# xiaosu-zhu/McQuic

Measured on AMD Instinct MI355X. Metric: images/sec encode+decode, 768x512 Kodak-shape batch, qp=2, higher is better.
Workload: dtype f32; 1 GPU; qp=2 reference model Compressor(128, 2, [8192, 2048, 512]), batch=32 768x512 random images per GPU, encode+decode tensor path (BASELINE configs[1]); images_per_gpu=32, parallelism=dp1 (independent image shards, no data-path collective)

## Files before the change

mcquic_amd/csrc/conv_launch.hip:

```cpp
#include <mutex>
#include <unordered_map>

#include "conv_instances.h"
#include "conv_sizes.h"
#include "conv_wino16.h"
#include "conv_head16.h"
#include "conv_t16.h"

namespace {

std::mutex g_sec_mu;
bool g_sec_trace = false;
std::unordered_map<const float*, unsigned> g_sec_used;
inline void sec_note(const mcq_conv_desc* descs, int nprob, unsigned bit) {
    if (!g_sec_trace) return;
    std::lock_guard<std::mutex> lock(g_sec_mu);
    for (int c = 0; c < nprob; ++c) g_sec_used[descs[c].w_packed] |= bit;
}

bool wino_shape(int Cout, int ksize, int stride, unsigned fl) {
    return ksize == 3 && stride == 1 && Cout % 64 == 0 && !(fl & (MCQ_CONV_SILU_IN | MCQ_CONV_SQUARE_IN));
}

inline bool post_fills_chip(long long tb, int row_tiles) { return tb * row_tiles >= 2048; }

int block_width_log2(int rows, int cols, int min_lg) {
    int best_log2 = 5; double best_util = -1.0;
    for (int lg = 5; lg >= min_lg; --lg) {
        const int bw = 1 << lg, bh = 32 >> lg;
        const double cover = (double)((rows + bh - 1) / bh * bh) * (double)((cols + bw - 1) / bw * bw);
        const double util = (double)rows * cols / cover;
        if (util > best_util + 1e-9) { best_util = util; best_log2 = lg; }
    }
    return best_log2;
}

template <class P> void conv_ptrs(P& a, const mcq_conv_desc* e, size_t sec4, size_t sec2) {
    a.x = e->x; a.wp = e->w_packed; a.wp64 = a.wp + sec4; a.wp32 = a.wp64 + sec2;
    a.bias = e->bias; a.y = e->y; a.y2 = e->y_silu; a.res = e->res; a.mul = e->mul; a.gid = e->gate_id;
}
template <class P> void w16_ptrs(P& a, const mcq_conv_desc* e) {
    a.x = e->x; a.wp = e->w_packed; a.bias = e->bias; a.y = e->y; a.y2 = e->y_silu; a.res = e->res;
}
void t16_ptrs(T16Ptrs& a, const mcq_conv_desc* e, size_t sec) {
    a.x = e->x; a.wp = e->w_packed + sec; a.bias = e->bias; a.y = e->y; a.y2 = e->y_silu; a.res = e->res; a.mul = e->mul;
}

int conv_validate(const mcq_conv_desc* d) {
    if (!d || !d->x || !d->w_packed || !d->y) return MCQ_EINVAL;
    if (d->N <= 0 || d->Cin <= 0 || d->H <= 0 || d->W <= 0 || d->Cout <= 0) return MCQ_EINVAL;
    if ((d->ksize != 1 && d->ksize != 3) || (d->stride != 1 && d->stride != 2)) return MCQ_EINVAL;
    if ((d->flags & MCQ_CONV_TAPS_LR) && (d->ksize != 3 || d->stride != 1 || (d->flags & (MCQ_CONV_WINOGRAD | MCQ_CONV_WINOGRAD2D | MCQ_CONV_WINOGRAD2D16 |
                                                                                    MCQ_CONV_SILU_IN | MCQ_CONV_SQUARE_IN)))) return MCQ_EINVAL;
    const unsigned fl = d->flags & ~(unsigned)MCQ_CONV_TAPS_LR;
    if (fl & MCQ_CONV_POST_MASK) {
        const unsigned post = fl & MCQ_CONV_POST_MASK;
        if ((post & (post - 1)) || !d->post_w || d->ksize != 3 || (d->flags & MCQ_CONV_TAPS_LR)) return MCQ_EINVAL;
        unsigned allowed = MCQ_CONV_POST_MASK | MCQ_CONV_SILU_IN;
        if (post == MCQ_CONV_POST_IGDN) allowed |= MCQ_CONV_SHUFFLE2;
        if (post == MCQ_CONV_POST_GATE) allowed |= MCQ_CONV_RESIDUAL | MCQ_CONV_DUAL_SILU;
        if (fl & ~allowed) return MCQ_EINVAL;
        if (d->Cout != ((fl & MCQ_CONV_SHUFFLE2) ? 512 : 128)) return MCQ_EINVAL;
        if (post == MCQ_CONV_POST_GATE && (!d->mul || !d->gate_id || d->stride != 1)) return MCQ_EINVAL;
    }
    if ((fl & MCQ_CONV_RESIDUAL) && !d->res) return MCQ_EINVAL;
    if ((fl & (MCQ_CONV_GDN | MCQ_CONV_IGDN | MCQ_CONV_GATE | MCQ_CONV_MUL | MCQ_CONV_DSILU_MUL)) && !d->mul) return MCQ_EINVAL;
    if ((fl & MCQ_CONV_GATE) && !d->gate_id) return MCQ_EINVAL;
    if ((fl & MCQ_CONV_DUAL_SILU) && (!d->y_silu || (fl & MCQ_CONV_SILU_OUT))) return MCQ_EINVAL;
    if (fl & (MCQ_CONV_GDN_BWD | MCQ_CONV_IGDN_BWD)) {
        if (!d->res || !d->mul || !d->y_silu || (fl & ~(unsigned)(MCQ_CONV_SQUARE_IN | MCQ_CONV_GDN_BWD | MCQ_CONV_IGDN_BWD)) ||
            (fl & MCQ_CONV_GDN_BWD && fl & MCQ_CONV_IGDN_BWD) || d->ksize != 1) return MCQ_EINVAL;
    }
    if (fl & MCQ_CONV_GATE_BWD) {
        if (!d->res || !d->mul || !d->y_silu || (fl & ~(unsigned)MCQ_CONV_GATE_BWD) || d->ksize != 1 || d->stride != 1) return MCQ_EINVAL;
    }
    if ((fl & MCQ_CONV_SILU_IN) && (fl & MCQ_CONV_SQUARE_IN)) return MCQ_EINVAL;
    if (fl & MCQ_CONV_SHUFFLE2) {
        if ((d->Cout & 3) || (fl & ~(unsigned)(MCQ_CONV_SHUFFLE2 | MCQ_CONV_SILU_IN | MCQ_CONV_SQUARE_IN | MCQ_CONV_WINOGRAD | MCQ_CONV_WINOGRAD2D | MCQ_CONV_WINOGRAD2D16 |
                                               MCQ_CONV_DSILU_MUL | MCQ_CONV_RESIDUAL | MCQ_CONV_POST_IGDN))) return MCQ_EINVAL;
        if ((fl & (MCQ_CONV_DSILU_MUL | MCQ_CONV_RESIDUAL)) && (fl & (MCQ_CONV_WINOGRAD | MCQ_CONV_WINOGRAD2D | MCQ_CONV_WINOGRAD2D16)))
            return MCQ_EINVAL;
    }
    if ((uint64_t)(d->Cin + 8) * d->H * d->W * 4ull >= 0x80000000ull) return MCQ_ETOOLARGE;
    return MCQ_OK;
}

bool t16_takes(int N, int Cin, int H, int W, int Cout, int ksize, int stride, unsigned fl, int nprob) {
    return N > 0 && H > 0 && W > 0 && nprob >= 1 && t16_shape(Cout, Cin, ksize) && stride == 1 && (fl & ~T16_FLAGS) == 0 &&
           t16_tiles((long long)N * H * W, Cout, nprob) <= T16_MAX_TILES &&
// ... 20 lines not shown
    for (int c = 1; c < MCQ_CONV_MAX_MULTI; ++c) conv_ptrs(k.alt[c - 1], descs + (c < nprob ? c : 0), sec4, sec2);

    if (fl & MCQ_CONV_WINOGRAD2D16) {
        if ((fl & (MCQ_CONV_WINOGRAD | MCQ_CONV_WINOGRAD2D)) || !wino_shape(d->Cout, d->ksize, d->stride, fl)) return MCQ_EINVAL;
        W16K w;
        w16_ptrs(w, d);
        for (int c = 1; c < W16_MAX_MULTI; ++c) w16_ptrs(w.alt[c - 1], descs + (c < nprob ? c : 0));
        w.nprob = nprob; w.N = d->N; w.Cin = d->Cin; w.H = d->H; w.W = d->W; w.Cout = d->Cout; w.Ho = k.Ho; w.Wo = k.Wo;
        w.flags = fl & ~(unsigned)MCQ_CONV_WINOGRAD2D16; w.res_scale = d->res_scale;
        return mcq_wino16_launch(w, stream);
    }
    if (fl & MCQ_CONV_WINOGRAD2D) {
        if ((fl & MCQ_CONV_WINOGRAD) || !wino_shape(d->Cout, d->ksize, d->stride, fl) || d->Cout % 128 != 0 || d->Cin % 8 != 0) return MCQ_EINVAL;
        if ((uint64_t)(d->Cin + 16) * d->H * d->W * 4ull >= 0x80000000ull) return MCQ_ETOOLARGE;
        k.TP = k.S * 16;
        k.wp32 = k.wp; k.wp64 = k.wp;
        for (int c = 1; c < MCQ_CONV_MAX_MULTI; ++c) { k.alt[c - 1].wp32 = k.alt[c - 1].wp; k.alt[c - 1].wp64 = k.alt[c - 1].wp; }
        const int Wt = (k.Wo + 1) / 2, Ht = (k.Ho + 1) / 2;
        const int best_log2 = block_width_log2(Ht, Wt, 0);
        k.bw_log2 = best_log2;
        k.nbx = (Wt + (1 << best_log2) - 1) >> best_log2;
        k.nby = (Ht + (32 >> best_log2) - 1) / (32 >> best_log2);
        const long long tbw = (long long)k.N * k.nbx * k.nby;
        if (tbw > 0x7fffffffLL) return MCQ_ETOOLARGE;
        k.total_blocks = (int)tbw;
        if ((uint64_t)d->Cout * (uint64_t)k.Ho * k.Wo * 4ull >= 0x80000000ull) return MCQ_ETOOLARGE;
        k.flags = fl & ~(unsigned)MCQ_CONV_WINOGRAD2D;
        return launch_wino2d(k, tbw, d->Cout / 128, (hipStream_t)stream);
    }
    if (fl & MCQ_CONV_WINOGRAD) {
        if (!wino_shape(d->Cout, d->ksize, d->stride, fl)) return MCQ_EINVAL;
        if ((uint64_t)(d->Cin + 16) * d->H * d->W * 4ull >= 0x80000000ull) return MCQ_ETOOLARGE;
        const int forced_mb = (d->tile & 0xff) >> 4;
        const int MBw = forced_mb == 2 || d->Cout % 128 != 0 ? 2 : 4;
        k.TP = k.S * 12;
        k.wp64 = k.wp + wino_section_floats(d->Cout, d->Cin, 4);
        k.wp32 = k.wp64;
        for (int c = 1; c < MCQ_CONV_MAX_MULTI; ++c) {
            k.alt[c - 1].wp64 = k.alt[c - 1].wp + wino_section_floats(d->Cout, d->Cin, 4);
            k.alt[c - 1].wp32 = k.alt[c - 1].wp64;
        }
        const int Wp = (k.Wo + 1) / 2;
        const int best_log2 = block_width_log2(k.Ho, Wp, 2);
        k.bw_log2 = best_log2;
        k.nbx = (Wp + (1 << best_log2) - 1) >> best_log2;
        k.nby = (k.Ho + (32 >> best_log2) - 1) / (32 >> best_log2);
        const long long tbw = (long long)k.N * k.nbx * k.nby;
        if (tbw > 0x7fffffffLL) return MCQ_ETOOLARGE;
        k.total_blocks = (int)tbw;
        const int co_tiles = (d->Cout + 32 * MBw - 1) / (32 * MBw);
        if ((uint64_t)co_tiles * 32u * (unsigned)MBw * (uint64_t)k.Ho * k.Wo * 4ull >= 0x80000000ull) return MCQ_ETOOLARGE;
        k.flags = fl & ~(unsigned)MCQ_CONV_WINOGRAD;
        return MBw == 4 ? launch_wino<4>(k, tbw, co_tiles, (hipStream_t)stream) : launch_wino<2>(k, tbw, co_tiles, (hipStream_t)stream);
    }

    if (d->tile == 0 && t16_takes(d->N, d->Cin, d->H, d->W, d->Cout, d->ksize, d->stride, fl, nprob)) {
        sec_note(descs, nprob, 8u);
        T16K t;
        const size_t sec = section_floats(d->Cout, d->Cin, 3, 4) + section_floats(d->Cout, d->Cin, 3, 2) + section_floats(d->Cout, d->Cin, 3, 1);
        for (int c = 0; c < MCQ_CONV_MAX_MULTI; ++c) t16_ptrs(t.p[c], descs + (c < nprob ? c : 0), sec);
        t.N = d->N; t.Cin = d->Cin; t.H = d->H; t.W = d->W; t.Cout = d->Cout; t.flags = fl; t.res_scale = d->res_scale;
        const dim3 grid((unsigned)(((long long)d->N * d->H * d->W + 15) / 16), (unsigned)(d->Cout / 16), (unsigned)nprob);
        if (d->Cin == 128) hipLaunchKernelGGL(conv_t16_kernel<8>, grid, dim3(256), 0, (hipStream_t)stream, t);
        else hipLaunchKernelGGL(conv_t16_kernel<4>, grid, dim3(256), 0, (hipStream_t)stream, t);
        return mcq_check_launch();
    }

    if (nprob == 1 && head16_shape(d->Cout, d->ksize) && d->stride == 1 && (d->tile & 0xff) == 0 &&
        (fl & ~(unsigned)(MCQ_CONV_SHUFFLE2 | MCQ_CONV_SILU_IN)) == 0) {
        if ((uint64_t)d->Cout * d->H * d->W * 4ull >= 0x80000000ull) return MCQ_ETOOLARGE;
        Head16K h;
        h.x = d->x; h.wp16 = d->w_packed + general_floats(d->Cout, d->Cin, d->ksize); h.bias = d->bias; h.y = d->y;
        h.N = d->N; h.Cin = d->Cin; h.H = d->H; h.W = d->W; h.Cout = d->Cout;
        h.S4 = (d->Cin + 3) / 4;
        h.gpr = (d->W + 15) / 16;
        h.total_groups = (long long)d->N * d->H * h.gpr;
        h.flags = fl;
        const long long waves = (h.total_groups + H16_NB - 1) / H16_NB;
        if ((waves + 3) / 4 > 0x7fffffffLL) return MCQ_ETOOLARGE;
        const dim3 grid((unsigned)((waves + 3) / 4));
        if (fl & MCQ_CONV_SILU_IN) hipLaunchKernelGGL(conv_head16_kernel<PRO_SILU>, grid, dim3(256), 0, (hipStream_t)stream, h);
        else hipLaunchKernelGGL(conv_head16_kernel<PRO_NONE>, grid, dim3(256), 0, (hipStream_t)stream, h);
        return mcq_check_launch();
    }

    const int best_log2 = block_width_log2(k.Ho, k.Wo, 2);
    k.bw_log2 = best_log2;
    const int bw = 1 << best_log2, bh = 32 >> best_log2;
    k.nbx = (k.Wo + bw - 1) / bw;
    k.nby = (k.Ho + bh - 1) / bh;
    const long long tb = (long long)k.N * k.nbx * k.nby;
    if (tb > 0x7fffffffLL) return MCQ_ETOOLARGE;
    k.total_blocks = (int)tb;

    const int co32 = (d->Cout + 31) / 32;
    int MB, NB, ksl = 0;
    bool dsilu41 = false;
    const int forced = d->tile & 0xff;
    if (forced) {
        MB = forced >> 4; NB = forced & 15; ksl = (d->tile >> 8) & 3;
        if ((MB != 1 && MB != 2 && MB != 4) || (NB != 1 && NB != 2 && NB != 4)) return MCQ_EINVAL;
    }
    else if (co32 == 1) {
        MB = 1; NB = (tb * nprob >= 4 * 2048) ? 4 : 2;
        if (d->Cin <= 64) {
            NB = (tb * nprob >= 16384) ? 2 : 1;
            while (ksl < 3 && (((tb + NB - 1) / NB * nprob) << ksl) < 1024) ++ksl;
        }
    }
    else if (co32 == 2 && ((tb + 1) / 2) * nprob < 2048 && d->ksize == 3) {
        MB = 1; NB = 1;
        while (ksl < 3 && ((tb * co32 * nprob) << ksl) < 1024) ++ksl;
    }
    else {
        static const int cand[3][2] = {{4, 2}, {2, 2}, {1, 1}};
        MB = 1; NB = 1;
        const bool rows64 = ((co32 + 3) / 4) * 4 > ((co32 + 1) / 2) * 2;
        for (int c = 0; c < 3; ++c) {
            const int mb = cand[c][0], nb = cand[c][1];
            if (mb > co32 || (mb == 4 && rows64)) continue;
            const long long tiles = ((tb + nb - 1) / nb) * ((co32 + mb - 1) / mb);
            MB = mb; NB = nb;
            if (tiles * 8 >= 1024) break;
        }
        const long long tiles1 = ((tb + NB - 1) / NB) * ((co32 + MB - 1) / MB);
        const long long tiles = tiles1 * nprob;
        while (ksl < 3 && (tiles << ksl) < 2048) ++ksl;
        int ksl1 = 0;
        while (ksl1 < 3 && (tiles1 << ksl1) < 2048) ++ksl1;
        if (MB == 4 && NB == 2 && ksl1 == 2 && tiles1 * 4 > 2048 && tiles1 * 4 <= 3072 && d->ksize == 3 &&
            k.S % 2 == 0 && (k.S >> 1) >= 8) { MB = 2; NB = 2; ksl = nprob >= 2 ? 0 : 1; }
        if (MB == 4 && NB == 2 && ksl == 3 && d->ksize == 3 && k.S % 4 == 0 && (k.S >> 2) >= 8) { NB = 1; ksl = 2; }
        else if (MB == 4 && NB == 2 && ksl == 1 && d->ksize == 3) { NB = 1; ksl = 0; }
        else if (MB == 4 && NB == 2 && ksl == 2 && nprob >= 2 && d->ksize == 3 && k.S % 2 == 0 && (k.S >> 1) >= 8) { MB = 2; ksl = 1; }
        else if (MB == 4 && NB == 2 && ksl == 0 && (fl & MCQ_CONV_DSILU_MUL) && d->ksize == 3) { NB = 1; dsilu41 = true; }
        if (d->ksize == 1 && d->stride == 1 && co32 >= 4) {
            const long long t41 = tb * ((co32 + 3) / 4) * nprob, t21 = tb * ((co32 + 1) / 2) * nprob;
            if (t41 >= 2048 && !rows64) { MB = 4; NB = 1; ksl = 0; }
            else if (t21 >= 2048) { MB = 2; NB = 1; ksl = 0; }
        }
    }
    if (fl & (MCQ_CONV_GDN_BWD | MCQ_CONV_IGDN_BWD)) {
        if (!(fl & MCQ_CONV_SQUARE_IN)) return MCQ_EINVAL;
        NB = 1; ksl = 0;
    }
    if (fl & MCQ_CONV_GATE_BWD) { NB = 1; ksl = 0; }
    int post = 0;
    if (fl & MCQ_CONV_POST_MASK) {
        if (nprob != 1 || lr4) return MCQ_EINVAL;
        if (!post_fills_chip(tb, (fl & MCQ_CONV_SHUFFLE2) ? 4 : 1) && forced != 0x41) return MCQ_EINVAL;
        MB = 4; NB = 1; ksl = 0; dsilu41 = false;
        post = (fl & MCQ_CONV_POST_GATE) ? 2 : 1;
        k.post_sub = (fl & MCQ_CONV_SHUFFLE2) ? 1 : 0;
    }
    const int pro = (fl & MCQ_CONV_SILU_IN) ? PRO_SILU : (fl & MCQ_CONV_SQUARE_IN) ? PRO_SQUARE : PRO_NONE;
    long long ptiles = (tb + NB - 1) / NB;
    const bool pair_ok = !post && !lr4 && MB == 4 && (NB == 2 || dsilu41) && ksl == 0 && d->ksize == 3 && d->stride == 1 && pro == PRO_NONE && (k.Wo & 1) == 0 &&
                         !(fl & ~(unsigned)(MCQ_CONV_SILU_OUT | MCQ_CONV_RESIDUAL | MCQ_CONV_DUAL_SILU | MCQ_CONV_DSILU_MUL | MCQ_CONV_SHUFFLE2));
    const bool pair = pair_ok && (d->tile & 0x400);
    if (pair) {
        const int Wp = k.Wo / 2;
        const int bl = block_width_log2(k.Ho, Wp, 2);
        const int pnbx = (Wp + (1 << bl) - 1) >> bl, pnby = (k.Ho + (32 >> bl) - 1) / (32 >> bl);
        const long long pt = (long long)k.N * pnbx * pnby;
        NB = 2; k.bw_log2 = bl; k.nbx = pnbx; k.nby = pnby; ptiles = pt; k.total_blocks = (int)pt;
    }
// ... 71 lines not shown
```

mcquic_amd/modules/compressor.py:

```python
from __future__ import annotations

import operator
from typing import List, Tuple

import torch
import torch.nn.functional as F
from torch import nn

from ..nn import AttentionBlock, ResidualBlock, ResidualBlockShuffle, ResidualBlockWithStride, conv3x3, pixelShuffle3x3
from ..utils.specification import FileHeader, ImageSize
from .quantizer import BaseQuantizer, ResidualBackwardQuantizer, UMGMQuantizer

from ..utils.specification import VERSION as __version__


_VERSION_OF = operator.attrgetter("_version")
_DATA_PTR_OF = operator.methodcaller("data_ptr")


def _forget_captures_hook(module, incompatible_keys):
    module._forgetCaptures()


class _GraphedCall:
# ... 162 lines not shown

    def encode(self, x: torch.Tensor) -> List[torch.Tensor]:
        self._check(x)
        if x.shape[0] == 0:
            return [c[:0] for c in self.encode(x.new_zeros((1,) + tuple(x.shape[1:])))]
        with torch.no_grad():
            if self._graphs is not None and x.is_cuda and not torch.cuda.is_current_stream_capturing():
                return self._graphed("encode", lambda t: self._quantizer.encode(self._encode_latent(t)), [x.contiguous()])
            return self._quantizer.encode(self._encode_latent(x))

    def decode(self, codes: List[torch.Tensor]) -> torch.Tensor:
        if codes[0].shape[0] == 0:
            return self.decode([c.new_zeros((1,) + tuple(c.shape[1:])) for c in codes])[:0]
        with torch.no_grad():
            if self._graphs is not None and codes[0].is_cuda and not torch.cuda.is_current_stream_capturing():
                return self._graphed("decode", lambda *c: self._decoder(self._quantizer.decode(list(c))), [c.contiguous() for c in codes])
            return self._decoder(self._quantizer.decode(codes))

    def compress(self, x: torch.Tensor) -> Tuple[List[torch.Tensor], List[List[bytes]], List[FileHeader]]:
        self._check(x)
        n, c, h, w = x.shape
        if n == 0:
            return self.encode(x), [], []
        with torch.no_grad():
            codes, binaries, codeSizes = self._quantizer.compress(self._encode_latent(x))
        header = [FileHeader(__version__, self._qp, codeSize, ImageSize(height=h, width=w, channel=c)) for codeSize in codeSizes]
        return codes, binaries, header

    def _checkHeaderGeometry(self, headers: List[FileHeader]):
        for header in headers:
            size, code = header.ImageSize, header.CodeSize
            if not (0 < int(size.height) <= (1 << 20) and 0 < int(size.width) <= (1 << 20)):
                raise RuntimeError("The header's image size is out of range.")
            base = self._padding._base
            ph, pw = -(-int(size.height) // base) * base, -(-int(size.width) // base) * base
            if len(code.heights) < 1 or int(code.heights[0]) * 16 != ph or int(code.widths[0]) * 16 != pw:
                raise RuntimeError(f"The header's code size {list(code.heights)} x {list(code.widths)} does not belong to a "
                                   f"{size.height} x {size.width} image.")

    def decompress(self, binaries: List[List[bytes]], headers: List[FileHeader]) -> torch.Tensor:
        if type(self)._encode_latent is BaseCompressor._encode_latent:
            self._checkHeaderGeometry(headers)
        with torch.no_grad():
            restored = self._decoder(self._quantizer.decompress(binaries, [header.CodeSize for header in headers]))
        imageSize = headers[0].ImageSize
        H, W = restored.shape[-2], restored.shape[-1]
        h, w = imageSize.height, imageSize.width
        cropTop, cropLeft = (H - h) // 2, (W - w) // 2
        return restored[..., cropTop:cropTop + h, cropLeft:cropLeft + w]


class Compressor(BaseCompressor):
    def __init__(self, channel: int, m: int, k: List[int], permutationRate: float = 0.0):
        encoder = nn.Sequential(
            conv3x3(3, channel, 2),
            ResidualBlock(channel, channel),
            ResidualBlockWithStride(channel, channel),
            AttentionBlock(channel),
            ResidualBlock(channel, channel),
            ResidualBlockWithStride(channel, channel),
            ResidualBlock(channel, channel))
        decoder = nn.Sequential(
            ResidualBlock(channel, channel),
            ResidualBlockShuffle(channel, channel),
            AttentionBlock(channel),
            ResidualBlock(channel, channel),
            ResidualBlockShuffle(channel, channel),
            ResidualBlock(channel, channel),
            pixelShuffle3x3(channel, 3, 2))
        quantizer = UMGMQuantizer(channel, m, k, permutationRate, {
            "latentStageEncoder": lambda: nn.Sequential(
                ResidualBlockWithStride(channel, channel), ResidualBlock(channel, channel), AttentionBlock(channel)),
            "quantizationHead": lambda: nn.Sequential(
                ResidualBlock(channel, channel), AttentionBlock(channel), conv3x3(channel, channel)),
            "latentHead": lambda: nn.Sequential(
                ResidualBlock(channel, channel), AttentionBlock(channel), conv3x3(channel, channel)),
            "restoreHead": lambda: nn.Sequential(
                AttentionBlock(channel), ResidualBlock(channel, channel), ResidualBlockShuffle(channel, channel)),
            "dequantizationHead": lambda: nn.Sequential(
                AttentionBlock(channel), conv3x3(channel, channel), ResidualBlock(channel, channel)),
            "sideHead": lambda: nn.Sequential(
                AttentionBlock(channel), conv3x3(channel, channel), ResidualBlock(channel, channel)),
        })
        super().__init__(encoder, quantizer, decoder)



class Neon(BaseCompressor):

    def __init__(self, channel: int, k: int, size: List[int], denseNorm: bool = False, *_, **__):
        quantizer = ResidualBackwardQuantizer(k, size, denseNorm)
        q = quantizer.channel
        encoder = nn.Sequential(
            conv3x3(3, channel),
            AttentionBlock(channel, 32, denseNorm),
            ResidualBlock(channel, channel, 32, denseNorm),
            ResidualBlock(channel, channel, 32, denseNorm),
            ResidualBlockWithStride(channel, channel, 2, 32, denseNorm),
            ResidualBlock(channel, channel, 32, denseNorm),
            ResidualBlockWithStride(channel, channel, 2, 32, denseNorm),
            ResidualBlock(channel, channel, 32, denseNorm),
            ResidualBlockWithStride(channel, channel, 2, 32, denseNorm),
            AttentionBlock(channel, 32, denseNorm),
            ResidualBlock(channel, 2 * channel, 32, denseNorm),
            ResidualBlock(2 * channel, 2 * channel, 32, denseNorm),
            ResidualBlock(2 * channel, 2 * channel, 32, denseNorm),
            ResidualBlock(2 * channel, 2 * channel, 32, denseNorm),
            ResidualBlock(2 * channel, q, 1, denseNorm),
            AttentionBlock(q, 1, denseNorm))
        decoder = nn.Sequential(
            AttentionBlock(q, 1, denseNorm),
            ResidualBlock(q, 2 * channel, 1, denseNorm),
            ResidualBlock(2 * channel, 2 * channel, 32, denseNorm),
            ResidualBlock(2 * channel, 2 * channel, 32, denseNorm),
            ResidualBlock(2 * channel, 2 * channel, 32, denseNorm),
            ResidualBlock(2 * channel, channel, 32, denseNorm),
            AttentionBlock(channel, 32, denseNorm),
            ResidualBlock(channel, channel, 32, denseNorm),
            ResidualBlockShuffle(channel, channel, 2, 32, denseNorm),
            ResidualBlock(channel, channel, 32, denseNorm),
            ResidualBlockShuffle(channel, channel, 2, 32, denseNorm),
            ResidualBlock(channel, channel, 32, denseNorm),
            ResidualBlockShuffle(channel, channel, 2, 32, denseNorm),
            ResidualBlock(channel, channel, 32, denseNorm),
            ResidualBlock(channel, channel, 32, denseNorm),
            AttentionBlock(channel, 32, denseNorm),
            conv3x3(channel, 3))
        super().__init__(encoder, quantizer, decoder)

    def _encode_latent(self, x: torch.Tensor, pad: bool = True) -> torch.Tensor:
        return self._encoder(self._padding(x) if pad else x)

    def residual_backward(self, code: torch.Tensor, level: int) -> torch.Tensor:
        with torch.no_grad():
            return self._quantizer.residual_backward(code, level)

    def residual_forward(self, code: torch.Tensor, formerLevel, level: int) -> torch.Tensor:
        with torch.no_grad():
            return self._quantizer.residual_forward(code, formerLevel, level)
```

mcquic_amd/modules/quantizer.py:

```python
from __future__ import annotations

import math
from typing import Callable, Dict, List, Optional, Union

import torch
from torch import nn

from .. import ops
from .entropyCoder import EntropyCoder, VariousMCoder

EPS = 1e-6
_TORCH_RAND = __import__("os").environ.get("MCQUIC_AMD_TORCH_RAND", "0") == "1"


class _CodebookCache:

    def __init__(self):
        self._packed: Optional[ops.PackedCodebook] = None
        self._key = None

    def invalidate(self):
        self._packed, self._key = None, None

    def get(self, codebook: torch.Tensor) -> ops.PackedCodebook:
# ... 93 lines not shown
        self._codebook = codebook
        self._cache = [cache]

    def forward(self, sample) -> torch.Tensor:
        if torch.is_tensor(sample):
            return sample
        index, hot = sample
        return ops.vq_dequant_soft(index, hot, self._cache[0].get(self._codebook))

    def decode(self, code: torch.Tensor, dual_silu: bool = False) -> torch.Tensor:
        return ops.vq_gather(code, self._cache[0].get(self._codebook), dual_silu=dual_silu)


class _quantizerEncoder(nn.Module):

    def __init__(self, quantizer, dequantizer, latentStageEncoder, quantizationHead, latentHead):
        super().__init__()
        self._quantizer = quantizer
        self._dequantizer = dequantizer
        self._latentStageEncoder = latentStageEncoder
        self._quantizationHead = quantizationHead
        self._latentHead = latentHead

    @property
    def Codebook(self):
        return self._quantizer._codebook

    def syncCodebook(self):
        self._quantizer.syncCodebook()

    def reAssignCodebook(self, freq: torch.Tensor) -> torch.Tensor:
        return self._quantizer.reAssignCodebook(freq)

    def encode(self, x: torch.Tensor):
        from ..nn import blocks
        z = self._latentStageEncoder(x)
        head = self._latentHead
        if head is None:
            return None, self._quantizer.encode(self._quantizationHead(z))
        if blocks.lockstep_ok([self._quantizationHead, head], [z, z]):
            last = len(head) - 1
            q, t = blocks.lockstep_infer([self._quantizationHead, head], [z, z], layers=last)
            code = self._quantizer.encode(self._quantizationHead[last](q))
        else:
            code = self._quantizer.encode(self._quantizationHead(z))
            t = z
            for i in range(len(head) - 1):
                t = head[i](t)
        deq = self._dequantizer.decode(code)
        return head[len(head) - 1](t, res=deq, res_scale=-1.0, dual_silu=True), code


    def _forward(self, x: torch.Tensor, freqEMA: torch.Tensor, uniforms=None, step=None):
        z = self._latentStageEncoder(x)
        if self._latentHead is None:
            q, code, logit = self._quantizer(self._quantizationHead(z), freqEMA, uniforms, step)
            return q, None, code, logit
        head = self._latentHead
        if torch.is_grad_enabled():
            from .. import autograd as AG
            hz, qin = AG.lockstep([head, self._quantizationHead], [z, z])
            q, code, logit = self._quantizer(qin, freqEMA, uniforms, step)
            residual, q = AG.sub_pass(hz, self._dequantizer(q))
            return q, residual, code, logit
        q, code, logit = self._quantizer(self._quantizationHead(z), freqEMA, uniforms, step)
        deq = self._dequantizer(q)
        t = z
        for i in range(len(head) - 1):
            t = head[i](t)
        return q, head[len(head) - 1](t, res=deq, res_scale=-1.0, dual_silu=True), code, logit

    def forward(self, x: torch.Tensor, freqEMA: torch.Tensor, uniforms=None, step=None):
        return self._forward(x, freqEMA, uniforms, step)


class _quantizerDecoder(nn.Module):

    def __init__(self, dequantizer, dequantizationHead, sideHead, restoreHead):
        super().__init__()
        self._dequantizer = dequantizer
        self._dequantizationHead = dequantizationHead
        self._sideHead = sideHead
        self._restoreHead = restoreHead

    def decode(self, code: torch.Tensor, formerLevel: Optional[torch.Tensor]):
        from ..nn import blocks
        deq = self._dequantizer.decode(code, dual_silu=True)
        if self._sideHead is None:
            return self._restoreHead(self._dequantizationHead(deq))
        if blocks.lockstep_ok([self._dequantizationHead, self._sideHead], [deq, formerLevel]):
            q, side = blocks.lockstep_infer([self._dequantizationHead, self._sideHead], [deq, formerLevel])
        else:
            q, side = self._dequantizationHead(deq), self._sideHead(formerLevel)
        return self._restoreHead(ops.add(q, side, dual_silu=True))


    def forward(self, q, formerLevel: Optional[torch.Tensor]):
        if self._sideHead is not None and torch.is_grad_enabled():
            from .. import autograd as AG
            x, side = AG.lockstep([self._dequantizationHead, self._sideHead], [self._dequantizer(q), formerLevel])
            return self._restoreHead(AG.add(x, side, dual_silu=True))
        from ..nn import blocks
        x = blocks.run_stack(self._dequantizationHead, self._dequantizer(q))
        if self._sideHead is not None:
            if torch.is_grad_enabled():
                from .. import autograd as AG
                x = AG.add(x, self._sideHead(formerLevel), dual_silu=True)
            else:
                x = ops.add(x, self._sideHead(formerLevel), dual_silu=True)
        return self._restoreHead(x)


class BaseQuantizer(nn.Module):

    def __init__(self, m: int, k: List[int]):
        super().__init__()
        self._entropyCoder = EntropyCoder(m, k)
        self._m = m
        self._k = k

    @property
    def CDFs(self):
        return self._entropyCoder.CDFs

    @property
    def NormalizedFreq(self):
        return self._entropyCoder.NormalizedFreq

    def _stepPrologue(self, x: torch.Tensor, uniforms):
        if not x.is_cuda:
            raise NotImplementedError(f"mcquic_amd: the training forward of {type(self).__name__} runs on a HIP device only (input on "
                                      f"{x.device}); there is no CPU / PyTorch fallback -- move the model and the batch to cuda")
        coder = self._entropyCoder
        want_rng = uniforms is None and not _TORCH_RAND
        return ops.vq_step_prologue(list(coder._freqEMA), EPS, want_rng, coder.countBuffer(x.device))

    def compress(self, x: torch.Tensor):
        codes = self.encode(x)
        binaries, codeSize = self._entropyCoder.compress(codes)
        return codes, binaries, codeSize

    def decompress(self, binaries, codeSize) -> torch.Tensor:
        return self.decode(self._entropyCoder.decompress(binaries, codeSize))


class UMGMQuantizer(BaseQuantizer):
    _components = ["latentStageEncoder", "quantizationHead", "latentHead", "dequantizationHead", "sideHead", "restoreHead"]

    def __init__(self, channel: int, m: int, k: Union[int, List[int]], permutationRate: float,
                 components: Dict[str, Callable[[], nn.Module]]):
        if isinstance(k, int):
            k = [k]
        super().__init__(m, k)
        lse, qh, lh, dqh, sh, rh = [components[key] for key in self._components]
        encoders, decoders = [], []
        for i, ki in enumerate(k):
            last = i == len(k) - 1
            codebook = nn.Parameter(nn.init.normal_(torch.empty(m, ki, channel // m), std=math.sqrt(2 / (5 * channel / m))))
            cache = _CodebookCache()
            quantizer = _multiCodebookQuantization(codebook, cache)
            dequantizer = _multiCodebookDeQuantization(codebook, cache)
            encoders.append(_quantizerEncoder(quantizer, dequantizer, lse(), qh(), None if last else lh()))
            decoders.append(_quantizerDecoder(dequantizer, dqh(), None if last else sh(), rh()))
        self._encoders = nn.ModuleList(encoders)
        self._decoders = nn.ModuleList(decoders)

# ... 283 lines not shown
```

mcquic_amd/nn/blocks.py:

```python
from __future__ import annotations

import os
from typing import Dict, Optional

import torch
from torch import nn

from .. import autograd as AG
from .. import ops
from .convs import conv1x1, conv3x3, pixelShuffle3x3
from .gdn import GenDivNorm, InvGenDivNorm

__all__ = ["ResidualBlockWithStride", "ResidualBlockShuffle", "ResidualBlock", "AttentionBlock"]

_BRANCH_STREAMS = os.environ.get("MCQUIC_AMD_BRANCH_STREAMS", "1") != "0"
_NORM_NODES = os.environ.get("MCQUIC_AMD_NORM_NODES", "1") != "0"
_BLOCK_NODES = os.environ.get("MCQUIC_AMD_BLOCK_NODES", "1") != "0"
_side_streams: Dict[tuple, "torch.cuda.Stream"] = {}
_MULTI_MAX_PIXELS = int(os.environ.get("MCQUIC_AMD_MULTI_MAX_PIXELS", str(64 * 1024)))
_FORK_MIN_PIXELS = int(os.environ.get("MCQUIC_AMD_FORK_MIN_PIXELS", str(128 * 1024)))


def _side_stream(main: "torch.cuda.Stream") -> "torch.cuda.Stream":
    key = (main.device.index, main.cuda_stream)
    st = _side_streams.get(key)
    if st is None:
        st = _side_streams[key] = torch.cuda.Stream(device=main.device)
    return st


class _fork:

    def __init__(self, x: torch.Tensor):
        self.on = _BRANCH_STREAMS and x.is_cuda and x.shape[0] * x.shape[-2] * x.shape[-1] >= _FORK_MIN_PIXELS
        if self.on:
            self.main = torch.cuda.current_stream(x.device)
            self.side = _side_stream(self.main)
        self.ctx = None

    def __enter__(self):
        if self.on:
            self.side.wait_stream(self.main)
            self.ctx = torch.cuda.stream(self.side)
            self.ctx.__enter__()
        return self

    def __exit__(self, *exc):
        if self.ctx is not None:
            self.ctx.__exit__(*exc)
        return False

    def join(self, t: torch.Tensor) -> torch.Tensor:
        if self.on:
            self.main.wait_stream(self.side)
            t.record_stream(self.main)
        return t


class _residulBlock(nn.Module):

    def __init__(self, act1: nn.Module, conv1: nn.Module, act2: nn.Module, conv2: nn.Module, skip: Optional[nn.Module]):
        super().__init__()
        self._branch = nn.Sequential(act1, conv1, act2, conv2)
        self._skip = skip


class GroupNorm(nn.GroupNorm):

    def forward(self, x: torch.Tensor) -> torch.Tensor:
        if self.training and torch.is_grad_enabled():
            return AG.group_norm(x, self)
        return ops.group_norm(x, self.weight, self.bias, self.num_groups, self.eps)


class ResidualBlock(_residulBlock):

    def __init__(self, inChannels: int, outChannels: int, groups: int = 1, denseNorm: bool = False):
        super().__init__(nn.SiLU(), conv3x3(inChannels, outChannels), GroupNorm(groups, outChannels) if denseNorm else nn.SiLU(),
                         conv3x3(outChannels, outChannels), conv1x1(inChannels, outChannels) if inChannels != outChannels else None)
        self.denseNorm = bool(denseNorm)

    def forward(self, x: torch.Tensor, res2: Optional[torch.Tensor] = None) -> torch.Tensor:
        if self.training and torch.is_grad_enabled():
            if self._skip is None and (_NORM_NODES or not self.denseNorm):
                return AG.residual_block(x, self)
            sx, x = AG.silu_fork(x)
            t = self._branch[1](sx)
            t = self._branch[2](t) if self.denseNorm else AG.silu(t)
            return self._branch[3](t, res=x if self._skip is None else self._skip(x), dual_silu=True)
        if self.denseNorm:
            t = self._branch[2](self._branch[1](x, silu_in=True))
        else:
            t = self._branch[1](x, silu_in=True, silu_out=True)
        identity = x if self._skip is None else self._skip(x)
        return self._branch[3](t, res=identity, dual_silu=True)


class ResidualBlockWithStride(_residulBlock):

    def __init__(self, inChannels: int, outChannels: int, stride: int = 2, groups: int = 1, denseNorm: bool = False):
        if stride != 2:
            raise NotImplementedError("only stride-2 ResidualBlockWithStride is on the path")
        super().__init__(nn.SiLU(), conv3x3(inChannels, outChannels, stride=stride), GenDivNorm(outChannels),
                         conv3x3(outChannels, outChannels), conv3x3(inChannels, outChannels, stride=stride))

    def forward(self, x: torch.Tensor) -> torch.Tensor:
        if self.training and torch.is_grad_enabled():
            if _BLOCK_NODES and self._branch[1].bias is not None:
                return AG.scale_block(x, self, up=False)
            sx, x = AG.silu_fork(x)
            t = self._branch[2](self._branch[1](sx))
            return self._branch[3](t, res=self._skip(x), dual_silu=True)
        with _fork(x) as f:
            identity = self._skip(x)
        c1, gdn = self._branch[1], self._branch[2]
        fuse = ops.post_ok(x, c1.packed(), c1.stride, "gdn")
        if fuse:
            t = c1(x, silu_in=True, post_gdn=gdn.packed_post(), tile=0 if fuse == 1 else fuse)
        else:
            t = gdn(c1(x, silu_in=True))
        return self._branch[3](t, res=f.join(identity), dual_silu=True)


class ResidualBlockShuffle(_residulBlock):

    def __init__(self, inChannels: int, outChannels: int, upsample: int = 2, groups: int = 1, denseNorm: bool = False):
        if upsample != 2:
            raise NotImplementedError("only 2x ResidualBlockShuffle is on the path")
        super().__init__(nn.SiLU(), pixelShuffle3x3(inChannels, outChannels, upsample), InvGenDivNorm(outChannels),
                         conv3x3(outChannels, outChannels), pixelShuffle3x3(inChannels, outChannels, upsample))

    def forward(self, x: torch.Tensor) -> torch.Tensor:
        if self.training and torch.is_grad_enabled():
            if _BLOCK_NODES and self._branch[1][0].bias is not None:
                return AG.scale_block(x, self, up=True)
            sx, x = AG.silu_fork(x)
            t = self._branch[2](self._branch[1](sx))
            return self._branch[3](t, res=self._skip(x), dual_silu=True)
        with _fork(x) as f:
            identity = self._skip(x)
        up, igdn = self._branch[1][0], self._branch[2]
        fuse = ops.post_ok(x, up.packed(), 1, "igdn", shuffle2=True)
        if fuse:
            t = ops.conv2d(x, up.packed_subpixel(), 1, silu_in=True, shuffle2=True, post_igdn=igdn.packed_post(), tile=0 if fuse == 1 else fuse)
        else:
            t = igdn(self._branch[1](x, silu_in=True))
        return self._branch[3](t, res=f.join(identity), dual_silu=True)


class AttentionBlock(nn.Module):

    def __init__(self, channel: int, groups: int = 1, denseNorm: bool = False):
        super().__init__()
        self._mainBranch = nn.Sequential(*[ResidualBlock(channel, channel, groups, denseNorm) for _ in range(3)])
        self._sideBranch = nn.Sequential(*[ResidualBlock(channel, channel, groups, denseNorm) for _ in range(3)],
                                         conv1x1(channel, channel))
        self.denseNorm = bool(denseNorm)

    def forward(self, x: torch.Tensor) -> torch.Tensor:
        if self.training and torch.is_grad_enabled():
            if self.denseNorm and not _NORM_NODES:
                xa, xb, xc = AG.fork(x, 3)
                return AG.gate(self._mainBranch(xa), self._sideBranch(xb), xc)
            return AG.attention_block(x, self)
        if ops._MULTI and not self.denseNorm and x.shape[0] * x.shape[2] * x.shape[3] <= _MULTI_MAX_PIXELS:
            a = b = x
            for i in range(3):
                m, sd = self._mainBranch[i]._branch, self._sideBranch[i]._branch
                ta, tb = ops.conv2d_multi([a, b], [m[1].packed(), sd[1].packed()], silu_in=True, silu_out=True)
                a, b = ops.conv2d_multi([ta, tb], [m[3].packed(), sd[3].packed()], per_problem=[dict(res=a), dict(res=b)], dual_silu=True)
            return self._sideBranch[3](b, gate_mul=a, gate_id=x, dual_silu=True)
        last, gate = self._sideBranch[2], self._sideBranch[3]
        fuse = 0 if (self.denseNorm or last._skip is not None) else ops.post_ok(x, last._branch[3].packed(), 1, "gate")
        if fuse:
            with _fork(x) as f:
                b = x
                for i in range(2):
                    b = self._sideBranch[i](b)
                t = last._branch[1](b, silu_in=True, silu_out=True)
            a = self._mainBranch(x)
            f.join(b)
            return ops.conv2d(f.join(t), last._branch[3].packed(), 1, res=b, post_gate=gate.packed_post(), gate_mul=a, gate_id=x, dual_silu=True, tile=0 if fuse == 1 else fuse)
        with _fork(x) as f:
            b = x
            for i in range(3):
                b = self._sideBranch[i](b)
        a = self._mainBranch(x)
        return self._sideBranch[3](f.join(b), gate_mul=a, gate_id=x, dual_silu=True)


def run_stack(stack, x: torch.Tensor) -> torch.Tensor:
    mods = list(stack)
    for i, m in enumerate(mods):
        nxt = mods[i + 1] if i + 1 < len(mods) else None
        if type(m).__name__ == "Conv2d" and isinstance(nxt, (_residulBlock, AttentionBlock)) and m.training and torch.is_grad_enabled():
            x = m(x, dual_silu=True)
        else:
            x = m(x)
    return x


def _infer_kind(m) -> Optional[str]:
    if isinstance(m, ResidualBlock) and m._skip is None and not m.denseNorm:
        return "rb"
    if isinstance(m, AttentionBlock) and not m.denseNorm:
        return "attn"
    if type(m).__name__ == "Conv2d" and m.kernelSize == 3 and m.stride == 1:
        return "conv"
    return None


def lockstep_ok(stacks, xs) -> bool:
    if not (ops._MULTI and len(stacks) >= 2):
        return False
    kinds = [[_infer_kind(m) for m in st] for st in stacks]
    if any(None in k for k in kinds) or any(k != kinds[0] for k in kinds[1:]):
        return False
    if any(x.shape != xs[0].shape for x in xs[1:]):
        return False
    return xs[0].shape[0] * xs[0].shape[2] * xs[0].shape[3] <= _MULTI_MAX_PIXELS


def lockstep_infer(stacks, xs, layers: Optional[int] = None):
    k = len(stacks)
    xs = list(xs)
    for li, layer in enumerate(zip(*stacks)):
        if layers is not None and li >= layers:
            break
        kind = _infer_kind(layer[0])
        if kind != "conv":
            twins = [ops.silu_twin(x) is not None for x in xs]
            if any(twins) and not all(twins):
                for x, has in zip(xs, twins):
                    if not has:
                        ops.set_silu_twin(x, ops.silu(x))
        if kind == "rb":
            ts = ops.conv2d_multi(xs, [m._branch[1].packed() for m in layer], silu_in=True, silu_out=True)
            xs = ops.conv2d_multi(ts, [m._branch[3].packed() for m in layer], per_problem=[dict(res=x) for x in xs], dual_silu=True)
        elif kind == "attn":
            a, b = list(xs), list(xs)
            for i in range(3):
                blocks = [m._mainBranch[i] for m in layer] + [m._sideBranch[i] for m in layer]
                ts = ops.conv2d_multi(a + b, [blk._branch[1].packed() for blk in blocks], silu_in=True, silu_out=True)
                ys = ops.conv2d_multi(ts, [blk._branch[3].packed() for blk in blocks], per_problem=[dict(res=t) for t in a + b], dual_silu=True)
                a, b = ys[:k], ys[k:]
            xs = ops.conv2d_multi(b, [m._sideBranch[3].packed() for m in layer],
                                  per_problem=[dict(gate_mul=ai, gate_id=xi) for ai, xi in zip(a, xs)], dual_silu=True)
        else:
            xs = ops.conv2d_multi(xs, [m.packed() for m in layer], dual_silu=True)
    return xs
```

profiles/kernel_stats.py:

```python
#!/usr/bin/env python3
import sqlite3
import sys

db = sqlite3.connect(sys.argv[1])
cur = db.cursor()
rows = cur.execute("select name, count(*), sum(end-start)/1e6, avg(end-start)/1e3, min(end-start)/1e3, max(end-start)/1e3 "
                   "from kernels group by name order by 3 desc").fetchall()
tot = sum(r[2] for r in rows)
print(f"# per kernel: total {tot:.2f} ms over {sum(r[1] for r in rows)} dispatches")
print(f"{'total_ms':>10} {'pct':>6} {'calls':>6} {'avg_us':>10} {'min_us':>10} {'max_us':>10}  kernel")
for r in rows:
    print(f"{r[2]:10.2f} {100 * r[2] / tot:6.2f} {r[1]:6d} {r[3]:10.1f} {r[4]:10.1f} {r[5]:10.1f}  {r[0][:120]}")
print("\n# conv / VQ / weight-gradient kernels by launch grid (workgroups x grid.y)")
rows = cur.execute("select name, grid_x, grid_y, workgroup_x, count(*), avg(end-start)/1e3, min(end-start)/1e3, sum(end-start)/1e6, "
                   "max(vgpr_count), max(accum_vgpr_count), grid_z from kernels where name like '%conv_mfma%' or name like '%conv_head16%' or name like '%conv_t16%' or name like '%conv_r16%' or name like '%vq_%' or name like '%wgrad%' "
                   "or name like '%fused_%' group by name, grid_x, grid_y, grid_z order by 8 desc").fetchall()
print(f"{'total_ms':>10} {'calls':>6} {'avg_us':>10} {'min_us':>10} {'wgs':>8} {'gy':>3} {'gz':>3} {'vgpr':>5}  kernel")
for r in rows:
    nm = r[0].replace("(anonymous namespace)::", "").replace("void ", "")
    print(f"{r[7]:10.2f} {r[4]:6d} {r[5]:10.1f} {r[6]:10.1f} {r[1] // max(r[3], 1):8d} {r[2]:3d} {r[10]:3d} {r[8]:5d}  {nm[:60]}")
```

Baseline: 261.8 images/s.

## Add dedicated stride-2 stem conv kernel and skip unread SiLU twin outputs

Adds a specialized MFMA kernel for the 3-input-channel stride-2 3x3 stem convolution. It processes 128-pixel strips per wave with weights held in registers and vectorized input loads, replacing the general implicit-GEMM path for that layer. Separately, it marks residual blocks whose SiLU twin output is never consumed (the last block in attention branches, the head tails before lockstep decode, and decoder[-2]) so the second SiLU output write is skipped. This saves memory bandwidth, but a twin that is actually read downstream would now be missing.

```diff
diff --git a/mcquic_amd/csrc/conv_launch.hip b/mcquic_amd/csrc/conv_launch.hip
--- a/mcquic_amd/csrc/conv_launch.hip
+++ b/mcquic_amd/csrc/conv_launch.hip
@@ -5,6 +5,7 @@
 #include "conv_sizes.h"
 #include "conv_wino16.h"
 #include "conv_head16.h"
+#include "conv_stem.h"
 #include "conv_t16.h"
 
 namespace {
@@ -191,6 +192,24 @@
         if (fl & MCQ_CONV_SILU_IN) hipLaunchKernelGGL(conv_head16_kernel<PRO_SILU>, grid, dim3(256), 0, (hipStream_t)stream, h);
         else hipLaunchKernelGGL(conv_head16_kernel<PRO_NONE>, grid, dim3(256), 0, (hipStream_t)stream, h);
         return mcq_check_launch();
+    }
+
+    if (nprob == 1 && stem_shape(d->Cin, d->Cout, d->ksize, d->stride) && (d->tile & 0xff) == 0 && !lr4 && (fl & ~STEM_FLAGS) == 0) {
+        if ((uint64_t)d->Cout * (uint64_t)k.Ho * k.Wo * 4ull >= 0x80000000ull) return MCQ_ETOOLARGE;
+        StemK t;
+        t.x = d->x; t.wp32 = k.wp32; t.bias = d->bias; t.y = d->y; t.y2 = d->y_silu;
+        t.N = d->N; t.Cin = d->Cin; t.H = d->H; t.W = d->W; t.Cout = d->Cout; t.Ho = k.Ho; t.Wo = k.Wo;
+        t.S = k.S;
+        t.spr = (k.Wo + STEM_PX - 1) / STEM_PX;
+        const long long strips = (long long)d->N * k.Ho * t.spr;
+        if (strips > 0x7fffffffLL) return MCQ_ETOOLARGE;
+        t.total_strips = (int)strips;
+        t.strips_per_wg = (int)((strips + 3071) / 3072);
+        const dim3 grid((unsigned)((strips + t.strips_per_wg - 1) / t.strips_per_wg), (unsigned)((d->Cout + 127) / 128));
+        const bool vec = k.Wo % 4 == 0 && d->W == 2 * k.Wo &&
+                         (((uintptr_t)d->x | (uintptr_t)d->y | (uintptr_t)d->y_silu) & 15u) == 0;
+        sec_note(descs, nprob, 4u);
+        return vec ? launch_stem<true>(t, fl, grid, (hipStream_t)stream) : launch_stem<false>(t, fl, grid, (hipStream_t)stream);
     }
 
     const int best_log2 = block_width_log2(k.Ho, k.Wo, 2);
diff --git a/mcquic_amd/csrc/conv_stem.h b/mcquic_amd/csrc/conv_stem.h
--- /dev/null
+++ b/mcquic_amd/csrc/conv_stem.h
@@ -0,0 +1,134 @@
+#pragma once
+
+namespace {
+
+struct StemK {
+    const float* x; const float* wp32; const float* bias; float* y; float* y2;
+    int N, Cin, H, W, Cout, Ho, Wo;
+    int S;
+    int spr;
+    int total_strips;
+    int strips_per_wg;
+};
+
+constexpr int STEM_PX = 128;
+constexpr unsigned STEM_FLAGS = MCQ_CONV_SILU_OUT | MCQ_CONV_DUAL_SILU;
+
+inline bool stem_shape(int Cin, int Cout, int ksize, int stride) { return ksize == 3 && stride == 2 && Cin <= 4 && Cout % 32 == 0; }
+
+template <bool VEC, unsigned EF>
+__global__ __launch_bounds__(256, 2) void conv_stem_kernel(StemK p) {
+    const int lane = threadIdx.x & 63;
+    const int wave = __builtin_amdgcn_readfirstlane((int)(threadIdx.x >> 6));
+    const int band = (int)blockIdx.y * 4 + wave;
+    if (band * 32 >= p.Cout) return;
+    const int hi = lane >> 5, j = lane & 31;
+    const int HW = p.H * p.W;
+    const unsigned HoWo = (unsigned)(p.Ho * p.Wo);
+    const unsigned plane_bytes = (unsigned)p.Cin * (unsigned)HW * 4u;
+    const unsigned slab_bytes = (unsigned)p.Cout * HoWo * 4u;
+
+    float A[2][9];
+    {
+        const unsigned steps = (unsigned)p.S * 9u;
+        const __amdgpu_buffer_rsrc_t wr = mcq_make_rsrc(mcq_uniform_ptr(p.wp32 + (size_t)band * steps * 64), steps * 256u);
+#pragma unroll
+        for (int s = 0; s < 2; ++s)
+#pragma unroll
+            for (int t = 0; t < 9; ++t) A[s][t] = mcq_buffer_load_s(wr, (unsigned)lane * 4u, (unsigned)(s * 9 + t) * 256u);
+    }
+    float bias16[16];
+    {
+        const __amdgpu_buffer_rsrc_t br = mcq_make_rsrc(mcq_uniform_ptr(p.bias ? p.bias : p.wp32), p.bias ? (unsigned)p.Cout * 4u : 0u);
+#pragma unroll
+        for (int r = 0; r < 16; ++r) bias16[r] = mcq_buffer_load_s(br, (unsigned)hi * 16u, (unsigned)(band * 32 + mcq_drow(r, 0)) * 4u);
+    }
+
+    for (int si = 0; si < p.strips_per_wg; ++si) {
+        const int strip = (int)blockIdx.x * p.strips_per_wg + si;
+        if (strip >= p.total_strips) break;
+        const int per_img = p.Ho * p.spr;
+        const int n = strip / per_img;
+        const int rem = strip - n * per_img;
+        const int yo = rem / p.spr;
+        const int x0 = (rem - yo * p.spr) * STEM_PX + 4 * j;
+        const __amdgpu_buffer_rsrc_t xr = mcq_make_rsrc(mcq_uniform_ptr(p.x + (size_t)n * p.Cin * HW), plane_bytes);
+
+        f32x16 acc[4];
+#pragma unroll
+        for (int nb = 0; nb < 4; ++nb)
+#pragma unroll
+            for (int r = 0; r < 16; ++r) acc[nb][r] = 0.0f;
+
+#pragma unroll
+        for (int s = 0; s < 2; ++s) {
+            if (s >= p.S) break;
+            const unsigned chan = (unsigned)((2 * s + hi) * HW) * 4u;
+            float in[3][9];
+#pragma unroll
+            for (int dy = 0; dy < 3; ++dy) {
+                const int yi = 2 * yo + dy - 1;
+                const bool row = yi >= 0 && yi < p.H;
+                if (VEC) {
+                    const bool v = row && x0 < p.Wo;
+                    const unsigned o = (unsigned)(yi * p.W + 2 * x0) * 4u + chan;
+                    const f32x4v lo = mcq_buffer_load4_s(xr, v ? o : MCQ_OOB, 0u), up = mcq_buffer_load4_s(xr, v ? o + 16u : MCQ_OOB, 0u);
+                    in[dy][0] = mcq_buffer_load(xr, v && x0 > 0 ? o - 4u : MCQ_OOB);
+#pragma unroll
+                    for (int e = 0; e < 4; ++e) { in[dy][1 + e] = lo[e]; in[dy][5 + e] = up[e]; }
+                } else {
+#pragma unroll
+                    for (int c = 0; c < 9; ++c) {
+                        const int xi = 2 * x0 + c - 1;
+                        const bool v = row && xi >= 0 && xi < p.W;
+                        in[dy][c] = mcq_buffer_load(xr, v ? (unsigned)(yi * p.W + xi) * 4u + chan : MCQ_OOB);
+                    }
+                }
+            }
+#pragma unroll
+            for (int tap = 0; tap < 9; ++tap)
+#pragma unroll
+                for (int nb = 0; nb < 4; ++nb)
+                    acc[nb] = __builtin_amdgcn_mfma_f32_32x32x2f32(A[s][tap], in[tap / 3][2 * nb + tap % 3], acc[nb], 0, 0, 0);
+        }
+
+        const size_t slab = (size_t)n * p.Cout * HoWo;
+        const __amdgpu_buffer_rsrc_t yr = mcq_make_rsrc(mcq_uniform_ptr(p.y + slab), slab_bytes);
+        const __amdgpu_buffer_rsrc_t y2r = mcq_make_rsrc(mcq_uniform_ptr(((EF & MCQ_CONV_DUAL_SILU) ? p.y2 : p.y) + slab), slab_bytes);
+        const unsigned pix = ((unsigned)(yo * p.Wo + x0) + 4u * (unsigned)hi * HoWo) * 4u;
+#pragma unroll
+        for (int r = 0; r < 16; ++r) {
+            const unsigned so = (unsigned)(band * 32 + mcq_drow(r, 0)) * HoWo * 4u;
+            float v[4], tw[4];
+#pragma unroll
+            for (int nb = 0; nb < 4; ++nb) {
+                v[nb] = acc[nb][r] + bias16[r];
+                if (EF & MCQ_CONV_SILU_OUT) v[nb] = mcq_silu(v[nb]);
+                if (EF & MCQ_CONV_DUAL_SILU) tw[nb] = mcq_silu(v[nb]);
+            }
+            if (VEC) {
+                const unsigned pvo = x0 < p.Wo ? pix : MCQ_OOB;
+                mcq_buffer_store4_s(f32x4v{v[0], v[1], v[2], v[3]}, yr, pvo, so);
+                if (EF & MCQ_CONV_DUAL_SILU) mcq_buffer_store4_s(f32x4v{tw[0], tw[1], tw[2], tw[3]}, y2r, pvo, so);
+            } else {
+#pragma unroll
+                for (int nb = 0; nb < 4; ++nb) {
+                    const unsigned pvo = x0 + nb < p.Wo ? pix + 4u * (unsigned)nb : MCQ_OOB;
+                    mcq_buffer_store_s(v[nb], yr, pvo, so);
+                    if (EF & MCQ_CONV_DUAL_SILU) mcq_buffer_store_s(tw[nb], y2r, pvo, so);
+                }
+            }
+        }
+    }
+}
+
+template <bool VEC>
+int launch_stem(const StemK& k, unsigned fl, dim3 grid, hipStream_t s) {
+    if (fl == 0u) hipLaunchKernelGGL((conv_stem_kernel<VEC, 0u>), grid, dim3(256), 0, s, k);
+    else if (fl == MCQ_CONV_SILU_OUT) hipLaunchKernelGGL((conv_stem_kernel<VEC, MCQ_CONV_SILU_OUT>), grid, dim3(256), 0, s, k);
+    else if (fl == MCQ_CONV_DUAL_SILU) hipLaunchKernelGGL((conv_stem_kernel<VEC, MCQ_CONV_DUAL_SILU>), grid, dim3(256), 0, s, k);
+    else return MCQ_EINVAL;
+    return mcq_check_launch();
+}
+
+}
diff --git a/mcquic_amd/modules/compressor.py b/mcquic_amd/modules/compressor.py
--- a/mcquic_amd/modules/compressor.py
+++ b/mcquic_amd/modules/compressor.py
@@ -268,6 +268,7 @@
             "sideHead": lambda: nn.Sequential(
                 AttentionBlock(channel), conv3x3(channel, channel), ResidualBlock(channel, channel)),
         })
+        decoder[-2].twin_unread = True
         super().__init__(encoder, quantizer, decoder)
 
 
diff --git a/mcquic_amd/modules/quantizer.py b/mcquic_amd/modules/quantizer.py
--- a/mcquic_amd/modules/quantizer.py
+++ b/mcquic_amd/modules/quantizer.py
@@ -199,6 +199,10 @@
         self._dequantizationHead = dequantizationHead
         self._sideHead = sideHead
         self._restoreHead = restoreHead
+        if sideHead is not None:
+            for head in (dequantizationHead, sideHead):
+                if isinstance(head, nn.Sequential) and hasattr(head[-1], "twin_unread"):
+                    head[-1].twin_unread = True
 
     def decode(self, code: torch.Tensor, formerLevel: Optional[torch.Tensor]):
         from ..nn import blocks
diff --git a/mcquic_amd/nn/blocks.py b/mcquic_amd/nn/blocks.py
--- a/mcquic_amd/nn/blocks.py
+++ b/mcquic_amd/nn/blocks.py
@@ -19,6 +19,7 @@
 _side_streams: Dict[tuple, "torch.cuda.Stream"] = {}
 _MULTI_MAX_PIXELS = int(os.environ.get("MCQUIC_AMD_MULTI_MAX_PIXELS", str(64 * 1024)))
 _FORK_MIN_PIXELS = int(os.environ.get("MCQUIC_AMD_FORK_MIN_PIXELS", str(128 * 1024)))
+_TRIM_TWINS = True
 
 
 def _side_stream(main: "torch.cuda.Stream") -> "torch.cuda.Stream":
@@ -79,6 +80,7 @@
         super().__init__(nn.SiLU(), conv3x3(inChannels, outChannels), GroupNorm(groups, outChannels) if denseNorm else nn.SiLU(),
                          conv3x3(outChannels, outChannels), conv1x1(inChannels, outChannels) if inChannels != outChannels else None)
         self.denseNorm = bool(denseNorm)
+        self.twin_unread = False
 
     def forward(self, x: torch.Tensor, res2: Optional[torch.Tensor] = None) -> torch.Tensor:
         if self.training and torch.is_grad_enabled():
@@ -93,7 +95,7 @@
         else:
             t = self._branch[1](x, silu_in=True, silu_out=True)
         identity = x if self._skip is None else self._skip(x)
-        return self._branch[3](t, res=identity, dual_silu=True)
+        return self._branch[3](t, res=identity, dual_silu=not (_TRIM_TWINS and self.twin_unread))
 
 
 class ResidualBlockWithStride(_residulBlock):
@@ -156,6 +158,8 @@
         self._sideBranch = nn.Sequential(*[ResidualBlock(channel, channel, groups, denseNorm) for _ in range(3)],
                                          conv1x1(channel, channel))
         self.denseNorm = bool(denseNorm)
+        self._mainBranch[2].twin_unread = True
+        self._sideBranch[2].twin_unread = True
 
     def forward(self, x: torch.Tensor) -> torch.Tensor:
         if self.training and torch.is_grad_enabled():
@@ -168,7 +172,8 @@
             for i in range(3):
                 m, sd = self._mainBranch[i]._branch, self._sideBranch[i]._branch
                 ta, tb = ops.conv2d_multi([a, b], [m[1].packed(), sd[1].packed()], silu_in=True, silu_out=True)
-                a, b = ops.conv2d_multi([ta, tb], [m[3].packed(), sd[3].packed()], per_problem=[dict(res=a), dict(res=b)], dual_silu=True)
+                a, b = ops.conv2d_multi([ta, tb], [m[3].packed(), sd[3].packed()], per_problem=[dict(res=a), dict(res=b)],
+                                        dual_silu=i < 2 or not _TRIM_TWINS)
             return self._sideBranch[3](b, gate_mul=a, gate_id=x, dual_silu=True)
         last, gate = self._sideBranch[2], self._sideBranch[3]
         fuse = 0 if (self.denseNorm or last._skip is not None) else ops.post_ok(x, last._branch[3].packed(), 1, "gate")
@@ -236,13 +241,15 @@
                         ops.set_silu_twin(x, ops.silu(x))
         if kind == "rb":
             ts = ops.conv2d_multi(xs, [m._branch[1].packed() for m in layer], silu_in=True, silu_out=True)
-            xs = ops.conv2d_multi(ts, [m._branch[3].packed() for m in layer], per_problem=[dict(res=x) for x in xs], dual_silu=True)
+            xs = ops.conv2d_multi(ts, [m._branch[3].packed() for m in layer], per_problem=[dict(res=x) for x in xs],
+                                  dual_silu=not (_TRIM_TWINS and all(m.twin_unread for m in layer)))
         elif kind == "attn":
             a, b = list(xs), list(xs)
             for i in range(3):
                 blocks = [m._mainBranch[i] for m in layer] + [m._sideBranch[i] for m in layer]
                 ts = ops.conv2d_multi(a + b, [blk._branch[1].packed() for blk in blocks], silu_in=True, silu_out=True)
-                ys = ops.conv2d_multi(ts, [blk._branch[3].packed() for blk in blocks], per_problem=[dict(res=t) for t in a + b], dual_silu=True)
+                ys = ops.conv2d_multi(ts, [blk._branch[3].packed() for blk in blocks], per_problem=[dict(res=t) for t in a + b],
+                                      dual_silu=i < 2 or not _TRIM_TWINS)
                 a, b = ys[:k], ys[k:]
             xs = ops.conv2d_multi(b, [m._sideBranch[3].packed() for m in layer],
                                   per_problem=[dict(gate_mul=ai, gate_id=xi) for ai, xi in zip(a, xs)], dual_silu=True)
diff --git a/profiles/kernel_stats.py b/profiles/kernel_stats.py
--- a/profiles/kernel_stats.py
+++ b/profiles/kernel_stats.py
@@ -13,7 +13,7 @@
     print(f"{r[2]:10.2f} {100 * r[2] / tot:6.2f} {r[1]:6d} {r[3]:10.1f} {r[4]:10.1f} {r[5]:10.1f}  {r[0][:120]}")
 print("\n# conv / VQ / weight-gradient kernels by launch grid (workgroups x grid.y)")
 rows = cur.execute("select name, grid_x, grid_y, workgroup_x, count(*), avg(end-start)/1e3, min(end-start)/1e3, sum(end-start)/1e6, "
-                   "max(vgpr_count), max(accum_vgpr_count), grid_z from kernels where name like '%conv_mfma%' or name like '%conv_head16%' or name like '%conv_t16%' or name like '%conv_r16%' or name like '%vq_%' or name like '%wgrad%' "
+                   "max(vgpr_count), max(accum_vgpr_count), grid_z from kernels where name like '%conv_mfma%' or name like '%conv_head16%' or name like '%conv_stem%' or name like '%conv_t16%' or name like '%conv_r16%' or name like '%vq_%' or name like '%wgrad%' "
                    "or name like '%fused_%' group by name, grid_x, grid_y, grid_z order by 8 desc").fetchall()
 print(f"{'total_ms':>10} {'calls':>6} {'avg_us':>10} {'min_us':>10} {'wgs':>8} {'gy':>3} {'gz':>3} {'vgpr':>5}  kernel")
 for r in rows:
```

Measured after the change: 262.9 images/s (median of 6 runs). No clear change (+0.4%).
